# yifangao112/DinoUNet

Hardware: AMD Instinct MI355X
Metric: 2D slices/sec training, dinounet_l 512x512 bf16 (higher is better)
Workload: dtype bf16; 1 GPU; dinounet_l train step (fwd+loss+bwd+clip+SGD), 512x512x3 slices, batch 8/GPU, frozen ViT + adapter + FAPM + U-Net decoder, random-init weights; global_batch=8, parallelism=dp1

## Files before the change

dinounet_amd/_build.py:

```python
import hashlib
import os
import subprocess
import sys

HERE = os.path.dirname(os.path.abspath(__file__))
CSRC = os.path.join(HERE, "csrc")
LIB = os.path.join(HERE, "libdinounet_hip.so")
SOURCES = ["gemm.hip", "gemm_bf16.hip", "gemm_glds.hip", "gemm_p8.hip", "gemm_rk.hip", "gemm_skinny.hip", "conv_halo.hip", "conv_strip.hip", "attention.hip", "norm.hip", "msda.hip", "elementwise.hip", "dwconv.hip", "loss.hip", "optim.hip", "augment.hip", "export.hip", "surface.hip", "cc.hip", "preprocess.hip", "dataload.hip", "fingerprint.hip"]
FLAGS = ["--offload-arch=gfx950", "-O3", "-std=c++17", "-fPIC", "-munsafe-fp-atomics", "-fno-gpu-rdc"]
if os.environ.get("DINOUNET_DEBUG_KNOBS") == "1":
    FLAGS.append("-DDU_DEBUG_KNOBS")
EXTRA_FLAGS = {"attention.hip": ["-mllvm", "-amdgpu-mfma-vgpr-form"], "conv_strip.hip": ["-mllvm", "-amdgpu-mfma-vgpr-form"]}
NO_SCRATCH = ("gemm_bf16.hip", "gemm_glds.hip", "gemm_p8.hip", "gemm_rk.hip", "gemm_skinny.hip", "conv_halo.hip", "conv_strip.hip", "attention.hip", "surface.hip", "dwconv.hip", "cc.hip", "preprocess.hip", "dataload.hip", "fingerprint.hip")
REMARK = "-Rpass-analysis=kernel-resource-usage"
import re as _re
_ABLATION = _re.compile(
    r"attn_fwd_kernelILi\d+ELb1EEE"
    r"|attn_fwd_w64_kernelILi\d+ELi\d+ELb1E"
    r"|attn_fwd_w64_kernelILi\d+ELi\d+ELb\dELi\d+ELi[1-9]\d*ELi\d+EEE"
    r"|attn_fwd_pipe_kernelILb1ELi\d+EEE|attn_fwd_pipe_kernelILb\dELi[1-9]\d*EEE")


def _digest():
    h = hashlib.sha256()
    for f in sorted(os.listdir(CSRC)) + ["../../include/dinounet_hip.h"]:
        p = os.path.join(CSRC, f)
        if os.path.isfile(p):
            h.update(f.encode())
            h.update(open(p, "rb").read())
    h.update(" ".join(FLAGS).encode())
    h.update(repr(sorted(EXTRA_FLAGS.items())).encode())
    return h.hexdigest()


def build(force: bool = False, verbose: bool = True) -> str:
    stamp = LIB + ".stamp"
    dig = _digest()
    if not force and os.path.exists(LIB) and os.path.exists(stamp) and open(stamp).read() == dig:
        return LIB
    hipcc = os.environ.get("HIPCC", "/opt/rocm/bin/hipcc")
    objs, procs = [], []
    os.makedirs(os.path.join(HERE, "build"), exist_ok=True)
    for s in SOURCES:
        o = os.path.join(HERE, "build", s.replace(".hip", ".o"))
        objs.append(o)
        cmd = [hipcc, *FLAGS, *EXTRA_FLAGS.get(s, []), *([REMARK] if s in NO_SCRATCH else []), "-c", os.path.join(CSRC, s), "-o", o]
# ... 31 lines not shown
```

dinounet_amd/csrc/norm.hip:

```cpp
#include "common.h"

int g_ln_rows2 = 1;

namespace {

template <typename TI, typename TO, int MAXV>
__global__ __launch_bounds__(256) void layernorm_fwd_kernel(const TI* __restrict__ x, long ldx, const float* __restrict__ w,
                                                            const float* __restrict__ b, TO* __restrict__ y, long ldy,
                                                            float* __restrict__ mean_out, float* __restrict__ rstd_out,
                                                            long rows, int D, float eps) {
  constexpr int VI = Elem<TI>::VEC;
  const int lane = threadIdx.x & 63;
  const long row = (long)blockIdx.x * 4 + (threadIdx.x >> 6);
  if (row >= rows) return;
  const int nvec = D / VI;
  float v[MAXV][VI];
  float s = 0.f;
#pragma unroll
  for (int i = 0; i < MAXV; i++) {
    int vi = lane + i * 64;
    if (vi < nvec) {
      Vec16<TI> t = as_vec<TI>(*(const uint4*)(x + row * ldx + (long)vi * VI));
#pragma unroll
      for (int j = 0; j < VI; j++) { v[i][j] = to_f32(t.v[j]); s += v[i][j]; }
    } else {
#pragma unroll
      for (int j = 0; j < VI; j++) v[i][j] = 0.f;
    }
  }
  const float mean = wave_sum(s) / (float)D;
  float s2 = 0.f;
#pragma unroll
  for (int i = 0; i < MAXV; i++) {
// ... 144 lines not shown
    const int vi = lane + i * 64;
#pragma unroll
    for (int j = 0; j < VI; j++) { wv[i][j] = vi < nvec ? w[vi * VI + j] : 0.f; sa[i][j] = 0.f; sb[i][j] = 0.f; }
  }
  const long r0 = (long)blockIdx.x * strip;
  const long r1 = r0 + strip < rows ? r0 + strip : rows;
  for (long row0 = r0 + wave; row0 < r1; row0 += 8) {
    uint4 rx[2][MAXV], rg[2][MAXV];
    float mu[2], rs[2];
#pragma unroll
    for (int u = 0; u < 2; u++) {
      const long row = row0 + 4 * u;
      const bool live = row < r1;
      mu[u] = live ? mean[row] : 0.f; rs[u] = live ? rstd[row] : 0.f;
#pragma unroll
      for (int i = 0; i < MAXV; i++) {
        const int vi = lane + i * 64;
        rx[u][i] = make_uint4(0, 0, 0, 0); rg[u][i] = make_uint4(0, 0, 0, 0);
        if (live && vi < nvec) {
          rx[u][i] = *(const uint4*)(x + row * (long)D + (long)vi * VI);
          rg[u][i] = *(const uint4*)(dy + row * (long)D + (long)vi * VI);
        }
      }
    }
#pragma unroll
    for (int u = 0; u < 2; u++) {
      const long row = row0 + 4 * u;
      if (row >= r1) break;
      float xh[MAXV][VI], g[MAXV][VI];
      float c1 = 0.f, c2 = 0.f;
#pragma unroll
      for (int i = 0; i < MAXV; i++) {
        const int vi = lane + i * 64;
        if (vi < nvec) {
          Vec16<T> tx = as_vec<T>(rx[u][i]);
          Vec16<T> tg = as_vec<T>(rg[u][i]);
#pragma unroll
          for (int j = 0; j < VI; j++) {
            const float gy = to_f32(tg.v[j]);
            xh[i][j] = (to_f32(tx.v[j]) - mu[u]) * rs[u];
            g[i][j] = gy * wv[i][j];
            c1 += g[i][j];
            c2 += g[i][j] * xh[i][j];
            sa[i][j] += gy * xh[i][j];
            sb[i][j] += gy;
          }
        }
      }
      c1 = wave_sum(c1) / (float)D;
      c2 = wave_sum(c2) / (float)D;
#pragma unroll
      for (int i = 0; i < MAXV; i++) {
        const int vi = lane + i * 64;
        if (vi < nvec) {
          Vec16<T> o;
          if (dres) {
            Vec16<T> tr = as_vec<T>(*(const uint4*)(dres + row * (long)D + (long)vi * VI));
#pragma unroll
            for (int j = 0; j < VI; j++) o.v[j] = from_f32<T>(rs[u] * (g[i][j] - c1 - xh[i][j] * c2) + to_f32(tr.v[j]));
          } else {
#pragma unroll
            for (int j = 0; j < VI; j++) o.v[j] = from_f32<T>(rs[u] * (g[i][j] - c1 - xh[i][j] * c2));
          }
          *(uint4*)(dx + row * (long)D + (long)vi * VI) = as_u4(o);
        }
      }
    }
  }
  if (wave > 0) {
#pragma unroll
    for (int i = 0; i < MAXV; i++) {
      const int vi = lane + i * 64;
      if (vi < nvec) {
#pragma unroll
        for (int j = 0; j < VI; j += 2)
          *(float4*)(ln_red + ((long)(wave - 1) * D + vi * VI + j) * 2) = make_float4(sa[i][j], sb[i][j], sa[i][j + 1], sb[i][j + 1]);
      }
    }
  }
  __syncthreads();
  if (wave == 0) {
#pragma unroll
    for (int i = 0; i < MAXV; i++) {
      const int vi = lane + i * 64;
      if (vi < nvec) {
#pragma unroll
        for (int j = 0; j < VI; j += 2) {
          float4 t = make_float4(sa[i][j], sb[i][j], sa[i][j + 1], sb[i][j + 1]);
#pragma unroll
          for (int q = 0; q < 3; q++) {
            const float4 u = *(const float4*)(ln_red + ((long)q * D + vi * VI + j) * 2);
            t.x += u.x; t.y += u.y; t.z += u.z; t.w += u.w;
          }
          *(float4*)(part + ((long)blockIdx.x * D + vi * VI + j) * 2) = t;
        }
      }
    }
// ... 492 lines not shown

template <typename T>
int ln_bwd_dispatch(const void* x, const void* dy, const float* w, const float* mean, const float* rstd, void* dx, float* dwdb,
                    long rows, int D, float* ws, long ws_elems, const void* dres, hipStream_t st) {
  const int nvec = D / Elem<T>::VEC;
  const int maxv = (nvec + 63) / 64;
  dim3 grid((unsigned)((rows + 3) / 4)), block(256);
  {
    static const bool off = DU_GETENV("DU_LN_BWD_FUSED") && atoi(DU_GETENV("DU_LN_BWD_FUSED")) == 0;
    const int STRIP = pick_strip(1, rows, D, Elem<T>::VEC);
    const long strips = (rows + STRIP - 1) / STRIP;
    const size_t lds = (size_t)3 * D * 2 * sizeof(float);
    if (!off && maxv <= 4 && ws && ws_elems >= strips * D * 2 && lds <= 64 * 1024) {
      return strip_launch(dwdb, ws, ws_elems, 1, strips, D, st, [&](float* part) {
#define LNF_LAUNCH(MV) hipLaunchKernelGGL((layernorm_bwd_fused_kernel<T, MV>), dim3((unsigned)strips), block, lds, st, (const T*)x, (const T*)dy, w, mean, rstd, (T*)dx, rows, D, (const T*)dres, STRIP, part)
        if (maxv <= 1) LNF_LAUNCH(1); else if (maxv <= 2) LNF_LAUNCH(2); else LNF_LAUNCH(4);
#undef LNF_LAUNCH
      }, 2);
    }
  }
#define LNB_LAUNCH(MV) hipLaunchKernelGGL((layernorm_bwd_dx_kernel<T, MV>), grid, block, 0, st, (const T*)x, (const T*)dy, w, mean, rstd, (T*)dx, rows, D, (const T*)dres)
  if (maxv <= 1) LNB_LAUNCH(1); else if (maxv <= 2) LNB_LAUNCH(2); else if (maxv <= 4) LNB_LAUNCH(4);
  else if (maxv <= 8) LNB_LAUNCH(8); else if (maxv <= 16) LNB_LAUNCH(16); else return DU_ERR_UNSUPPORTED;
#undef LNB_LAUNCH
  const int STRIP = pick_strip(1, rows, D, Elem<T>::VEC);
  long strips = (rows + STRIP - 1) / STRIP;
  return strip_launch(dwdb, ws, ws_elems, 1, strips, D, st, [&](float* part) {
    hipLaunchKernelGGL(layernorm_bwd_wb_kernel<T>, dim3((unsigned)strips), block, 0, st, (const T*)x, (const T*)dy, mean, rstd, dwdb, rows, D, STRIP, part);
  }, (ws && ws_elems >= (long)strips * D * 2) ? 2 : 0);
}

}

extern "C" int du_layernorm_fwd(int in_dtype, int out_dtype, const void* x, int64_t ldx, const float* w, const float* b, void* y,
                                int64_t ldy, float* mean_out, float* rstd_out, int64_t rows, int D, float eps, void* stream) {
  hipStream_t st = (hipStream_t)stream;
  if (rows <= 0 || D <= 0 || !x || !y || !w || !b) return DU_ERR_BAD_ARG;
  const int vi = in_dtype == DU_BF16 ? 8 : 4;
  if (D % vi || ldx % vi) return DU_ERR_BAD_ARG;
  if (in_dtype == DU_F32 && out_dtype == DU_F32) return ln_fwd_dispatch<float, float>(x, ldx, w, b, y, ldy, mean_out, rstd_out, rows, D, eps, st);
  if (in_dtype == DU_F32 && out_dtype == DU_BF16) return ln_fwd_dispatch<float, bf16_t>(x, ldx, w, b, y, ldy, mean_out, rstd_out, rows, D, eps, st);
  if (in_dtype == DU_BF16 && out_dtype == DU_BF16) return ln_fwd_dispatch<bf16_t, bf16_t>(x, ldx, w, b, y, ldy, mean_out, rstd_out, rows, D, eps, st);
  if (in_dtype == DU_BF16 && out_dtype == DU_F32) return ln_fwd_dispatch<bf16_t, float>(x, ldx, w, b, y, ldy, mean_out, rstd_out, rows, D, eps, st);
  return DU_ERR_BAD_ARG;
}

extern "C" int du_strip_finalize(const float* part, float* out, int G, int strips, int C, void* stream) {
  hipStream_t st = (hipStream_t)stream;
  if (!part || !out || G <= 0 || strips <= 0 || C <= 0) return DU_ERR_BAD_ARG;
  if ((long)G * C * 2 >= 4096) {
    const int chunks = (C * 2 + 31) / 32;
    hipLaunchKernelGGL(finalize_kernel<32>, dim3((unsigned)(G * chunks)), dim3(256), 0, st, part, out, G, strips, C * 2, 0);
  } else {
    const int chunks = (C * 2 + 3) / 4;
    hipLaunchKernelGGL(finalize_kernel<4>, dim3((unsigned)(G * chunks)), dim3(256), 0, st, part, out, G, strips, C * 2, 0);
  }
  return du_check_launch();
}

extern "C" int64_t du_reduce_ws_elems(int dtype, int G, int64_t P, int C) {
  const int v = dtype == DU_BF16 ? 8 : 4;
  if (G <= 0 || P <= 0 || C <= 0 || C % v) return 0;
  const int STRIP = pick_strip(G, P, C, v);
  return (int64_t)G * ((P + STRIP - 1) / STRIP) * C * 2;
}

// ... 180 lines not shown
```

dinounet_amd/dinov3/adapter.py:

```python
import math
from functools import partial

import torch
from torch import nn

from .. import ops
from .._lib import ACT_GELU, ACT_NONE, ACT_RELU


def _act_dtype(module):
    return getattr(module, "_act_dtype", torch.bfloat16)


class MSDeformAttn(nn.Module):

    def __init__(self, d_model=256, n_levels=4, n_heads=8, n_points=4, ratio=1.0):
        super().__init__()
        if d_model % n_heads != 0:
            raise ValueError("d_model must be divisible by n_heads, but got {} and {}".format(d_model, n_heads))
        self.im2col_step = 64
        self.d_model, self.n_levels, self.n_heads, self.n_points, self.ratio = d_model, n_levels, n_heads, n_points, ratio
        self.sampling_offsets = nn.Linear(d_model, n_heads * n_levels * n_points * 2)
        self.attention_weights = nn.Linear(d_model, n_heads * n_levels * n_points)
        self.value_proj = nn.Linear(d_model, int(d_model * ratio))
        self.output_proj = nn.Linear(int(d_model * ratio), d_model)
        self._reset_parameters()

    def _reset_parameters(self):
        nn.init.constant_(self.sampling_offsets.weight.data, 0.0)
        thetas = torch.arange(self.n_heads, dtype=torch.float32) * (2.0 * math.pi / self.n_heads)
        grid_init = torch.stack([thetas.cos(), thetas.sin()], -1)
        grid_init = (grid_init / grid_init.abs().max(-1, keepdim=True)[0]).view(self.n_heads, 1, 1, 2).repeat(
            1, self.n_levels, self.n_points, 1)
        for i in range(self.n_points):
            grid_init[:, :, i, :] *= i + 1
        with torch.no_grad():
            self.sampling_offsets.bias = nn.Parameter(grid_init.view(-1))
        nn.init.constant_(self.attention_weights.weight.data, 0.0)
        nn.init.constant_(self.attention_weights.bias.data, 0.0)
        nn.init.xavier_uniform_(self.value_proj.weight.data)
        nn.init.constant_(self.value_proj.bias.data, 0.0)
        nn.init.xavier_uniform_(self.output_proj.weight.data)
        nn.init.constant_(self.output_proj.bias.data, 0.0)

    def forward(self, query, reference_points, input_flatten, input_spatial_shapes, input_level_start_index,
                input_padding_mask=None, residual=None):
        assert input_padding_mask is None and self.n_levels == 1 and len(input_spatial_shapes) == 1
        N, Lq, _ = query.shape
        _, S, _ = input_flatten.shape
        Hs, Ws = input_spatial_shapes[0]
        assert Hs * Ws == S
        M, P = self.n_heads, self.n_points
        value = ops.linear(input_flatten, self.value_proj.weight, self.value_proj.bias)
        value = value.view(N, S, M, value.shape[-1] // M)
        loc, attn = ops.offsets_prep(query, self.sampling_offsets.weight, self.attention_weights.weight, self.sampling_offsets.bias,
                                     self.attention_weights.bias, reference_points, Lq, M, P, Hs, Ws)
        shapes, lsi = _level_tensors(Hs, Ws, query.device)
        out = ops.msda(value, shapes, lsi, loc.view(N, Lq, M, 1, P, 2), attn.view(N, Lq, M, 1, P))
        return ops.linear(out, self.output_proj.weight, self.output_proj.bias, residual=residual)


_LEVEL_CACHE = {}


def _level_tensors(Hs, Ws, device):
    key = (Hs, Ws, str(device))
    if key not in _LEVEL_CACHE:
        _LEVEL_CACHE[key] = (torch.tensor([[Hs, Ws]], dtype=torch.long, device=device),
                             torch.zeros(1, dtype=torch.long, device=device))
    return _LEVEL_CACHE[key]


class DWConv(nn.Module):
    def __init__(self, dim=768):
        super().__init__()
        self.dwconv = nn.Conv2d(dim, dim, 3, 1, 1, bias=True, groups=dim)


class ConvFFN(nn.Module):

    def __init__(self, in_features, hidden_features=None, out_features=None, drop=0.0):
        super().__init__()
        out_features = out_features or in_features
        hidden_features = hidden_features or in_features
        self.fc1 = nn.Linear(in_features, hidden_features)
        self.dwconv = DWConv(hidden_features)
        self.act = nn.GELU()
        self.fc2 = nn.Linear(hidden_features, out_features)
        self.drop = nn.Dropout(drop)

    def forward(self, x, H, W, residual=None, row_scale=None):
        h = ops.linear(x, self.fc1.weight, self.fc1.bias)
        h = ops.dwconv_tokens(h, self.dwconv.dwconv.weight, self.dwconv.dwconv.bias, H, W, ACT_GELU)
        return ops.linear(h, self.fc2.weight, self.fc2.bias, residual=residual, row_scale=row_scale, rs_rows=x.shape[1])


class DropPath(nn.Module):
    def __init__(self, drop_prob=0.0):
        super().__init__()
        self.drop_prob = drop_prob
        self.pinned_mask = None
        self.predrawn = None

    def mask(self, B, device):
        if self.drop_prob == 0.0 or not self.training:
            return None
        if self.pinned_mask is not None:
            return self.pinned_mask.to(device=device, dtype=torch.float32)
        if self.predrawn is not None and self.predrawn.shape[0] == B:
            m, self.predrawn = self.predrawn, None
            return m
        keep = 1 - self.drop_prob
        m = torch.empty(B, device=device, dtype=torch.float32).bernoulli_(keep)
        if keep > 0.0:
            m.div_(keep)
        return m


class Extractor(nn.Module):

    def __init__(self, dim, num_heads=6, n_points=4, n_levels=1, deform_ratio=1.0, with_cffn=True, cffn_ratio=0.25, drop=0.0,
                 drop_path=0.0, norm_layer=partial(nn.LayerNorm, eps=1e-6), with_cp=False):
        super().__init__()
        self.query_norm = norm_layer(dim)
        self.feat_norm = norm_layer(dim)
        self.attn = MSDeformAttn(d_model=dim, n_levels=n_levels, n_heads=num_heads, n_points=n_points, ratio=deform_ratio)
        self.with_cffn = with_cffn
        self.with_cp = with_cp
        if with_cffn:
            self.ffn = ConvFFN(in_features=dim, hidden_features=int(dim * cffn_ratio), drop=drop)
            self.ffn_norm = norm_layer(dim)
            self.drop_path = DropPath(drop_path) if drop_path > 0.0 else nn.Identity()

    def forward(self, query, reference_points, feat, spatial_shapes, level_start_index, H, W):
        qn, qres = ops.layer_norm_res(query, self.query_norm.weight, self.query_norm.bias, self.query_norm.eps)
        fn = ops.layer_norm(feat, self.feat_norm.weight, self.feat_norm.bias, self.feat_norm.eps)
        query = self.attn(qn, reference_points, fn, spatial_shapes, level_start_index, None, residual=qres)
        if self.with_cffn:
            f, fres = ops.layer_norm_res(query, self.ffn_norm.weight, self.ffn_norm.bias, self.ffn_norm.eps)
            mask = self.drop_path.mask(query.shape[0], query.device) if isinstance(self.drop_path, DropPath) else None
            query = self.ffn(f, H, W, residual=fres, row_scale=mask)
        return query


class InteractionBlockWithCls(nn.Module):

    def __init__(self, dim, num_heads=6, n_points=4, norm_layer=partial(nn.LayerNorm, eps=1e-6), drop=0.0, drop_path=0.0,
                 with_cffn=True, cffn_ratio=0.25, init_values=0.0, deform_ratio=1.0, extra_extractor=False, with_cp=False):
        super().__init__()
        mk = lambda: Extractor(dim=dim, n_levels=1, num_heads=num_heads, n_points=n_points, norm_layer=norm_layer,
                               deform_ratio=deform_ratio, with_cffn=with_cffn, cffn_ratio=cffn_ratio, drop=drop,
                               drop_path=drop_path, with_cp=with_cp)
        self.extractor = mk()
        self.extra_extractors = nn.Sequential(*[mk() for _ in range(2)]) if extra_extractor else None

    def forward(self, x, c, ref, shapes, H_c, W_c):
        c = self.extractor(c, ref, x, shapes, None, H_c, W_c)
        if self.extra_extractors is not None:
            for ex in self.extra_extractors:
                c = ex(c, ref, x, shapes, None, H_c, W_c)
        return c


class SpatialPriorModule(nn.Module):

    def __init__(self, inplanes=64, embed_dim=384, with_cp=False):
        super().__init__()
        bn = nn.SyncBatchNorm
        self.stem = nn.Sequential(
            nn.Conv2d(3, inplanes, kernel_size=3, stride=2, padding=1, bias=False), bn(inplanes), nn.ReLU(inplace=True),
            nn.Conv2d(inplanes, inplanes, kernel_size=3, stride=1, padding=1, bias=False), bn(inplanes), nn.ReLU(inplace=True),
            nn.Conv2d(inplanes, inplanes, kernel_size=3, stride=1, padding=1, bias=False), bn(inplanes), nn.ReLU(inplace=True),
            nn.MaxPool2d(kernel_size=3, stride=2, padding=1))
        self.conv2 = nn.Sequential(nn.Conv2d(inplanes, 2 * inplanes, 3, 2, 1, bias=False), bn(2 * inplanes), nn.ReLU(inplace=True))
# ... 187 lines not shown
```

dinounet_amd/ops.py:

```python
import ctypes as C
import math
import os
import weakref

import torch

from . import _lib
from ._lib import (ACT_GELU, ACT_LEAKY, ACT_NONE, ACT_RELU, ACT_SWIGLU, DU_BF16, DU_F32, IM2COL_COL, IM2COL_ROW, PLAIN_COL,
                   PLAIN_ROW, STORE_MSDA_PREP, STORE_PIXEL_SHUFFLE2, STORE_QKV_HEADS, STORE_QKV_ROPE, STORE_SLABS, ConvGeom, GemmArgs)

__all__ = ["mm", "linear", "conv2d", "conv_transpose2x2", "norm_act", "layer_norm", "msda", "dwconv3x3",
           "maxpool3x3s2", "bilinear_add", "bilinear_resize", "squeeze_excite", "dice_ce_loss", "dice_ce_masked_loss", "dice_bce_loss",
           "labels_to_regions", "val_dice_ce", "val_dice_bce"]


def _code(dt):
    if dt == torch.bfloat16:
        return DU_BF16
    if dt == torch.float32:
        return DU_F32
    raise RuntimeError(f"dinounet_amd: unsupported dtype {dt} (bf16 / fp32 only)")


def _req(*ts):
# ... 1695 lines not shown
                kw = dict(dtype=DU_BF16, out_dtype=DU_F32, a_mode=PLAIN_ROW, b_mode=PLAIN_ROW, M=rows, N=Nw, K=K, A=xm.data_ptr(), lda=lda,
                          B=wq.data_ptr(), ldb=ldb, Cmat=loc.data_ptr(), ldc=Nw, bias=_dp(bq), store_mode=STORE_MSDA_PREP, ps=(Hs, Ws, Lq),
                          rope=(ref.data_ptr(), None, 0, 1.0), c2=attn.data_ptr())
                if gemm_route(**kw) == 3:
                    gemm_raw(**kw)
                    return None
            raw = mm(xm, wq, bias=bq, out_dtype=torch.float32)
            _, _, ld = _rows2d(raw)
            _lib.check(_lib.lib().du_msda_prep(_code(raw.dtype), _p(raw), ld, _p(ref), _p(loc), _p(attn), rows, Lq, M, P, Hs, Ws, _st()),
                       "du_msda_prep")
            return None

        assert w1.shape[0] + w2.shape[0] == ncol
        _linear_cat_fwd(ctx, x, w1, w2, b1, b2, torch.float32, product=product)
        xs, wq = ctx.lc_saved
        ctx.lc_saved = None
        ctx.save_for_backward(xs, wq, attn)
        ctx.prep = (M, P, Hs, Ws, ncol)
        return loc, attn

    @staticmethod
    def backward(ctx, gloc, gattn):
        x, wq, attn = ctx.saved_tensors
        M, P, Hs, Ws, ncol = ctx.prep
        rows = attn.shape[0]
        graw = torch.empty((rows, ncol), dtype=x.dtype, device=attn.device)
        _lib.check(_lib.lib().du_msda_prep_bwd(_code(x.dtype), _p(attn), _p(gloc.contiguous()), _p(gattn.contiguous()), _p(graw), ncol, rows,
                                               M, P, Hs, Ws, _st()), "du_msda_prep_bwd")
        return (*_linear_cat_bwd(ctx, graw, x, wq), None, None, None, None, None, None)


def offsets_prep(x, w1, w2, b1, b2, ref, Lq, M, P, Hs, Ws):
    return _OffsetsPrep.apply(x.reshape(-1, x.shape[-1]), w1, w2, b1, b2, ref, Lq, M, P, Hs, Ws)


def _dwconv_fwd(ctx, x, w, bias, geom, act):
    x = x.contiguous()
    Cc = w.shape[0]
    wf = _f32(w).view(Cc, 9)
    y = torch.empty_like(x)
    z = torch.empty_like(x) if act != ACT_NONE else None
    ld, bs, B, H, W, pyramid = geom
    _lib.check(_lib.lib().du_dwconv3x3_fwd(_code(x.dtype), _p(x), _p(wf), _p(_f32(bias)), _p(y), _p(z), ld, bs, B, H, W, Cc, pyramid, act, _st()),
               "du_dwconv3x3_fwd")
    ctx.save_for_backward(x, wf, z)
    ctx.conf = (geom, act, bias is not None)
    return y


def _dwconv_bwd(ctx, dy):
    x, wf, z = ctx.saved_tensors
    (ld, bs, B, H, W, pyramid), act, has_bias = ctx.conf
    Cc = wf.shape[0]
    L = _lib.lib()
    code = _code(x.dtype)
    dy = dy.contiguous()
    dz = torch.empty_like(dy) if act != ACT_NONE else None
    dx = torch.empty_like(x)
    dw = torch.empty((Cc, 9), dtype=torch.float32, device=x.device)
    db = torch.empty(Cc, dtype=torch.float32, device=x.device) if has_bias else None
    n = int(L.du_dwconv3x3_bwd_ws_elems(code, ld, bs, B, H, W, Cc, pyramid, act))
    ws = torch.empty(max(n, 1), dtype=torch.float32, device=x.device)
    _lib.check(L.du_dwconv3x3_bwd(code, _p(z), _p(dy), _p(x), _p(wf), _p(dx), _p(dw), _p(db), _p(dz), ld, bs, B, H, W, Cc, pyramid, act,
                                  _p(ws), n, _st()), "du_dwconv3x3_bwd")
    return dx, dw.view(Cc, 1, 3, 3), db

# ... 579 lines not shown
```

include/dinounet_hip.h:

```cpp
#ifndef DINOUNET_HIP_H
#define DINOUNET_HIP_H

#include <stdint.h>

#ifdef __cplusplus
extern "C" {
#endif

#define DU_OK 0
#define DU_ERR_BAD_ARG (-1)
#define DU_ERR_UNSUPPORTED (-2)
#define DU_ERR_LAUNCH (-3)

#define DU_F32 0
#define DU_BF16 1

#define DU_PLAIN_ROW 0
#define DU_PLAIN_COL 1
#define DU_IM2COL_ROW 2
#define DU_IM2COL_COL 3

#define DU_ACT_NONE 0
#define DU_ACT_GELU 1
#define DU_ACT_RELU 2
// ... 66 lines not shown
} du_tn_job;
int du_gemm_tn_group_legal(const du_tn_job* job);
int du_gemm_tn_group(const du_tn_job* jobs, int njobs, void* stream);

int du_conv3x3_halo(const void* x, int64_t ldx, const void* x2, int64_t ldx2, int C1, int Cin, int Cout, int B, int H, int W,
                    const void* w, const float* bias, void* y, int64_t ldy, float* stats_part, void* stream);
int du_conv3x3_plan_describe(const void* x, int64_t ldx, const void* x2, int64_t ldx2, int C1, int Cin, int Cout, int B, int H, int W,
                             const void* w, const void* y, int64_t ldy, int want_stats, int64_t* out, int n);
int du_conv3x3_halo_parts(int C1, int Cin, int Cout, int B, int H, int W);
int du_conv3x3_strip(const void* x, int64_t ldx, const void* x2, int64_t ldx2, int C1, int Cin, int Cout, int B, int H, int W,
                     const void* w, const float* bias, void* y, int64_t ldy, float* stats_part, void* stream);
int du_conv3x3_wgrad_halo(const void* x, int64_t ldx, const void* x2, int64_t ldx2, int C1, int Cin, int Cout, int B, int H, int W,
                          const void* dy, int64_t lddy, float* part, float* dw, int with_db, void* stream);
int du_conv3x3_wgrad_plan_describe(const void* x, int64_t ldx, const void* x2, int64_t ldx2, int C1, int Cin, int Cout, int B, int H, int W,
                                   const void* dy, int64_t lddy, int64_t* out, int n);
int du_conv3x3_wgrad_halo_blocks(int C1, int Cin, int Cout, int B, int H, int W);
int du_strip_finalize(const float* part, float* out, int G, int strips, int C, void* stream);

int du_qkv_rope_split(int dtype, const void* qkv, void* q, void* k, void* v, const float* sin_t, const float* cos_t,
                      int B, int N, int Npad, int H, int Dh, int prefix, float qscale, void* stream);
int du_qkv_rope_split_rows(int dtype, const void* qkv_rows, void* q, void* k, void* v, const float* sin_t, const float* cos_t, int B, int N,
                           int Npad, int H, int Dh, int prefix, float qscale, int64_t m_begin, int m_count, void* stream);
int du_qkv_rope_inplace(int dtype, void* q, void* k, const float* sin_t, const float* cos_t, int B, int N, int Npad, int H, int Dh,
                        int prefix, float qscale, int64_t m_limit, void* stream);
int du_attention_fwd(const void* q, const void* k, const void* v, void* out, int B, int H, int N, int Npad, int Dh,
                     void* stream);
int du_softmax_rows_f32(float* x, int64_t rows, int cols, int64_t ld, void* stream);

int du_layernorm_fwd(int in_dtype, int out_dtype, const void* x, int64_t ldx, const float* w, const float* b, void* y,
                     int64_t ldy, float* mean_out, float* rstd_out, int64_t rows, int D, float eps, void* stream);
int64_t du_reduce_ws_elems(int dtype, int G, int64_t pix_per_group, int C);
int du_layernorm_bwd(int dtype, const void* x, const void* dy, const float* w, const float* mean, const float* rstd,
                     void* dx, float* dwdb, int64_t rows, int D, float* ws, int64_t ws_elems, const void* dres, void* stream);

int du_chan_stats(int dtype, const void* x, int64_t ldx, float* sums, int G, int64_t pix_per_group, int C, float* ws,
                  int64_t ws_elems, void* stream);
int du_colsum(int dtype, const void* x, int64_t ldx, float* out, int64_t rows, int C, float* ws, int64_t ws_elems, void* stream);
int du_chan_dot(int dtype, const void* a, int64_t lda, const void* b, int64_t ldb, float* sums, int G, int64_t pix_per_group, int C,
                float* ws, int64_t ws_elems, void* stream);
int du_norm_stats_finalize(const float* sums, float count, float eps, float* mean, float* rstd, int G, int C, float* run_mean,
                           float* run_var, float momentum, void* stream);
int du_norm_param_grads(const float* bsums, float* dw, float* db, int G, int C, void* stream);
int du_chan_stats_norm(int dtype, const void* x, int64_t ldx, float* sums, int G, int64_t pix_per_group, int C, float* ws, int64_t ws_elems,
                       float count, float eps, float* mean, float* rstd, float* run_mean, float* run_var, float momentum, void* stream);
int du_strip_finalize_norm(const float* part, float* sums, int G, int strips, int C, float count, float eps, float* mean, float* rstd,
                           float* run_mean, float* run_var, float momentum, void* stream);
int du_norm_act_bwd_stats_grads(int dtype, const void* x, int64_t ldx, const void* dy, int64_t lddy, const float* mean, const float* rstd,
                                const float* w, const float* b, float* bsums, float* dw, float* db, int G, int64_t pix_per_group, int C,
                                int act, float* ws, int64_t ws_elems, void* stream);
int du_norm_act_fwd(int dtype, const void* x, int64_t ldx, void* y, int64_t ldy, const float* mean, const float* rstd,
                    const float* w, const float* b, int G, int64_t pix_per_group, int C, int act, void* stream);
int du_norm_act_bwd_stats(int dtype, const void* x, int64_t ldx, const void* dy, int64_t lddy, const float* mean,
                          const float* rstd, const float* w, const float* b, float* bsums, int G, int64_t pix_per_group,
                          int C, int act, float* ws, int64_t ws_elems, void* stream);
int du_norm_act_bwd_dx(int dtype, const void* x, int64_t ldx, const void* dy, int64_t lddy, void* dx, int64_t lddx,
                       const float* mean, const float* rstd, const float* w, const float* b, const float* bsums, int G,
                       int64_t pix_per_group, int C, int act, float count, int use_batch_stats, void* stream);

int du_msda_forward(int dtype, const void* value, const int64_t* spatial_shapes, const int64_t* level_start_index,
                    const float* sampling_loc, const float* attn_weight, void* out, int N, int S, int M, int D, int L,
                    int Lq, int P, void* stream);
int64_t du_msda_bwd_ws_elems(int N, int S, int M, int D, int L, int Lq, int P);
int du_msda_backward(int dtype, const void* value, const int64_t* spatial_shapes, const int64_t* level_start_index,
                     const float* sampling_loc, const float* attn_weight, const void* grad_out, float* grad_value,
                     float* grad_sampling_loc, float* grad_attn_weight, int N, int S, int M, int D, int L, int Lq, int P,
                     float* ws, int64_t ws_elems, void* stream);
// ... 186 lines not shown
```

Before: 310.2 slices/s.

## Fuse LayerNorm backward with preceding linear dgrad GEMM for adapter blocks

Adds a fused kernel that computes the input gradient dy = G·W of a small-K linear layer with MFMA into LDS and immediately applies LayerNorm backward on those rows, avoiding writing and re-reading the dy intermediate in global memory. New autograd functions combine LayerNorm with the following linear or offsets-prep projection so the backward can use this path when D=1024 and K<=256 in bf16. The kernel prefetches the next rows' x/dres while processing and reduces weight-grad partials per workgroup. It adds complexity and shape restrictions, with fallback to the separate GEMM plus LN-backward path otherwise.

```diff
diff --git a/dinounet_amd/_build.py b/dinounet_amd/_build.py
--- a/dinounet_amd/_build.py
+++ b/dinounet_amd/_build.py
@@ -6,12 +6,12 @@
 HERE = os.path.dirname(os.path.abspath(__file__))
 CSRC = os.path.join(HERE, "csrc")
 LIB = os.path.join(HERE, "libdinounet_hip.so")
-SOURCES = ["gemm.hip", "gemm_bf16.hip", "gemm_glds.hip", "gemm_p8.hip", "gemm_rk.hip", "gemm_skinny.hip", "conv_halo.hip", "conv_strip.hip", "attention.hip", "norm.hip", "msda.hip", "elementwise.hip", "dwconv.hip", "loss.hip", "optim.hip", "augment.hip", "export.hip", "surface.hip", "cc.hip", "preprocess.hip", "dataload.hip", "fingerprint.hip"]
+SOURCES = ["gemm.hip", "gemm_bf16.hip", "gemm_glds.hip", "gemm_p8.hip", "gemm_rk.hip", "gemm_skinny.hip", "conv_halo.hip", "conv_strip.hip", "attention.hip", "norm.hip", "norm_gemm.hip", "msda.hip", "elementwise.hip", "dwconv.hip", "loss.hip", "optim.hip", "augment.hip", "export.hip", "surface.hip", "cc.hip", "preprocess.hip", "dataload.hip", "fingerprint.hip"]
 FLAGS = ["--offload-arch=gfx950", "-O3", "-std=c++17", "-fPIC", "-munsafe-fp-atomics", "-fno-gpu-rdc"]
 if os.environ.get("DINOUNET_DEBUG_KNOBS") == "1":
     FLAGS.append("-DDU_DEBUG_KNOBS")
 EXTRA_FLAGS = {"attention.hip": ["-mllvm", "-amdgpu-mfma-vgpr-form"], "conv_strip.hip": ["-mllvm", "-amdgpu-mfma-vgpr-form"]}
-NO_SCRATCH = ("gemm_bf16.hip", "gemm_glds.hip", "gemm_p8.hip", "gemm_rk.hip", "gemm_skinny.hip", "conv_halo.hip", "conv_strip.hip", "attention.hip", "surface.hip", "dwconv.hip", "cc.hip", "preprocess.hip", "dataload.hip", "fingerprint.hip")
+NO_SCRATCH = ("gemm_bf16.hip", "gemm_glds.hip", "gemm_p8.hip", "gemm_rk.hip", "gemm_skinny.hip", "conv_halo.hip", "conv_strip.hip", "attention.hip", "norm_gemm.hip", "surface.hip", "dwconv.hip", "cc.hip", "preprocess.hip", "dataload.hip", "fingerprint.hip")
 REMARK = "-Rpass-analysis=kernel-resource-usage"
 import re as _re
 _ABLATION = _re.compile(
diff --git a/dinounet_amd/csrc/ln_bwd_row.h b/dinounet_amd/csrc/ln_bwd_row.h
--- /dev/null
+++ b/dinounet_amd/csrc/ln_bwd_row.h
@@ -0,0 +1,37 @@
+#pragma once
+#include "common.h"
+
+template <typename T>
+__device__ __forceinline__ void ln_bwd_row_terms(const uint4& rx, const uint4& rg, float mu, float rs, const float (&wv)[Elem<T>::VEC],
+                                                 float (&xh)[Elem<T>::VEC], float (&g)[Elem<T>::VEC], float& c1, float& c2,
+                                                 float (&sa)[Elem<T>::VEC], float (&sb)[Elem<T>::VEC]) {
+#pragma clang fp contract(off)
+  constexpr int VI = Elem<T>::VEC;
+  const Vec16<T> tx = as_vec<T>(rx);
+  const Vec16<T> tg = as_vec<T>(rg);
+#pragma unroll
+  for (int j = 0; j < VI; j++) {
+    const float gy = to_f32(tg.v[j]);
+    xh[j] = (to_f32(tx.v[j]) - mu) * rs;
+    g[j] = gy * wv[j];
+    c1 = c1 + g[j];
+    c2 = __builtin_fmaf(g[j], xh[j], c2);
+    sa[j] = __builtin_fmaf(gy, xh[j], sa[j]);
+    sb[j] = sb[j] + gy;
+  }
+}
+
+template <typename T, bool RES>
+__device__ __forceinline__ uint4 ln_bwd_row_dx(const float (&xh)[Elem<T>::VEC], const float (&g)[Elem<T>::VEC], float c1, float c2, float rs,
+                                               const uint4& rr) {
+#pragma clang fp contract(off)
+  constexpr int VI = Elem<T>::VEC;
+  const Vec16<T> tr = as_vec<T>(rr);
+  Vec16<T> o;
+#pragma unroll
+  for (int j = 0; j < VI; j++) {
+    const float t = __builtin_fmaf(-xh[j], c2, g[j] - c1);
+    o.v[j] = from_f32<T>(RES ? __builtin_fmaf(rs, t, to_f32(tr.v[j])) : rs * t);
+  }
+  return as_u4(o);
+}
diff --git a/dinounet_amd/csrc/norm.hip b/dinounet_amd/csrc/norm.hip
--- a/dinounet_amd/csrc/norm.hip
+++ b/dinounet_amd/csrc/norm.hip
@@ -1,4 +1,5 @@
 #include "common.h"
+#include "ln_bwd_row.h"
 
 int g_ln_rows2 = 1;
 
@@ -209,20 +210,7 @@
 #pragma unroll
       for (int i = 0; i < MAXV; i++) {
         const int vi = lane + i * 64;
-        if (vi < nvec) {
-          Vec16<T> tx = as_vec<T>(rx[u][i]);
-          Vec16<T> tg = as_vec<T>(rg[u][i]);
-#pragma unroll
-          for (int j = 0; j < VI; j++) {
-            const float gy = to_f32(tg.v[j]);
-            xh[i][j] = (to_f32(tx.v[j]) - mu[u]) * rs[u];
-            g[i][j] = gy * wv[i][j];
-            c1 += g[i][j];
-            c2 += g[i][j] * xh[i][j];
-            sa[i][j] += gy * xh[i][j];
-            sb[i][j] += gy;
-          }
-        }
+        if (vi < nvec) ln_bwd_row_terms<T>(rx[u][i], rg[u][i], mu[u], rs[u], wv[i], xh[i], g[i], c1, c2, sa[i], sb[i]);
       }
       c1 = wave_sum(c1) / (float)D;
       c2 = wave_sum(c2) / (float)D;
@@ -230,16 +218,10 @@
       for (int i = 0; i < MAXV; i++) {
         const int vi = lane + i * 64;
         if (vi < nvec) {
-          Vec16<T> o;
-          if (dres) {
-            Vec16<T> tr = as_vec<T>(*(const uint4*)(dres + row * (long)D + (long)vi * VI));
-#pragma unroll
-            for (int j = 0; j < VI; j++) o.v[j] = from_f32<T>(rs[u] * (g[i][j] - c1 - xh[i][j] * c2) + to_f32(tr.v[j]));
-          } else {
-#pragma unroll
-            for (int j = 0; j < VI; j++) o.v[j] = from_f32<T>(rs[u] * (g[i][j] - c1 - xh[i][j] * c2));
-          }
-          *(uint4*)(dx + row * (long)D + (long)vi * VI) = as_u4(o);
+          uint4 o;
+          if (dres) o = ln_bwd_row_dx<T, true>(xh[i], g[i], c1, c2, rs[u], *(const uint4*)(dres + row * (long)D + (long)vi * VI));
+          else o = ln_bwd_row_dx<T, false>(xh[i], g[i], c1, c2, rs[u], make_uint4(0, 0, 0, 0));
+          *(uint4*)(dx + row * (long)D + (long)vi * VI) = o;
         }
       }
     }
@@ -798,6 +780,12 @@
 
 }
 
+int du_norm_finalize_planar(const float* part, float* out, int strips, int C, hipStream_t st) {
+  if ((long)C * 2 >= 4096) hipLaunchKernelGGL(finalize_kernel<32>, dim3((unsigned)((C * 2 + 31) / 32)), dim3(256), 0, st, part, out, 1, strips, C * 2, 2);
+  else hipLaunchKernelGGL(finalize_kernel<4>, dim3((unsigned)((C * 2 + 3) / 4)), dim3(256), 0, st, part, out, 1, strips, C * 2, 2);
+  return du_check_launch();
+}
+
 extern "C" int du_layernorm_fwd(int in_dtype, int out_dtype, const void* x, int64_t ldx, const float* w, const float* b, void* y,
                                 int64_t ldy, float* mean_out, float* rstd_out, int64_t rows, int D, float eps, void* stream) {
   hipStream_t st = (hipStream_t)stream;
diff --git a/dinounet_amd/csrc/norm_gemm.hip b/dinounet_amd/csrc/norm_gemm.hip
--- /dev/null
+++ b/dinounet_amd/csrc/norm_gemm.hip
@@ -0,0 +1,279 @@
+#include "common.h"
+#include "ln_bwd_row.h"
+#include "norm_gemm_plan.h"
+
+int du_norm_finalize_planar(const float* part, float* out, int strips, int C, hipStream_t st);
+
+namespace {
+
+constexpr int LP_D = 1024;
+constexpr int LP_BM = 64;
+constexpr int LP_WGS = 256;
+constexpr int LP_DY_BYTES = LP_BM * LP_D * 2;
+
+struct LnProdParams {
+  const bf16_t* x; const bf16_t* G; const bf16_t* Wt; const bf16_t* dres; bf16_t* dx;
+  const float* w; const float* mean; const float* rstd; float* part;
+  long rows, ldg, ldw;
+  int rows_per_wg;
+};
+
+template <int KT>
+__global__ __launch_bounds__(512) void layernorm_bwd_prod_kernel(const LnProdParams P) {
+  constexpr int K = 64 * KT, KC = K / 8, D = LP_D, VI = 8, MAXV = 2;
+  extern __shared__ __attribute__((aligned(16))) unsigned char lp_smem[];
+  bf16_t* dyl = (bf16_t*)lp_smem;
+  bf16_t* gl = (bf16_t*)(lp_smem + LP_DY_BYTES);
+  const int tid = threadIdx.x, lane = tid & 63;
+  const int wave = __builtin_amdgcn_readfirstlane(tid >> 6);
+  const int lr = lane & 31, lh = lane >> 5;
+  const long r_begin = (long)blockIdx.x * P.rows_per_wg;
+  const long r_end = r_begin + P.rows_per_wg < P.rows ? r_begin + P.rows_per_wg : P.rows;
+  float wv[MAXV][VI], sa[MAXV][VI], sb[MAXV][VI];
+#pragma unroll
+  for (int i = 0; i < MAXV; i++) {
+    const int vi = lane + i * 64;
+#pragma unroll
+    for (int j = 0; j < VI; j++) { wv[i][j] = P.w[vi * VI + j]; sa[i][j] = 0.f; sb[i][j] = 0.f; }
+  }
+  const int wperm = 16 * ((lr >> 2) & 1) + 4 * (lr >> 3) + (lr & 3);
+  const int ldg = (int)P.ldg, ldw = (int)P.ldw;
+  const unsigned woff = (unsigned)(wperm * ldw + 8 * lh);
+  uint4 nx[2][MAXV], nr[2][MAXV];
+  float nmu[2], nrs[2];
+  auto request = [&](long b0, int nrows, int l0, bool with_dres) {
+#pragma unroll
+    for (int u = 0; u < 2; u++) {
+      const int l = l0 + 8 * u;
+      const bool live = l < nrows;
+      const long row = b0 + l;
+      nmu[u] = live ? P.mean[row] : 0.f; nrs[u] = live ? P.rstd[row] : 0.f;
+#pragma unroll
+      for (int i = 0; i < MAXV; i++) {
+        const int vi = lane + i * 64;
+        nx[u][i] = make_uint4(0, 0, 0, 0);
+        if (live) nx[u][i] = *(const uint4*)((P.x + row * (long)D) + (unsigned)(vi * VI));
+        if (with_dres) {
+          nr[u][i] = make_uint4(0, 0, 0, 0);
+          if (live && P.dres) nr[u][i] = *(const uint4*)((P.dres + row * (long)D) + (unsigned)(vi * VI));
+        }
+      }
+    }
+  };
+  auto process = [&](long b0, int nrows, int l0, const uint4 (&rx)[2][MAXV], const uint4 (&rr)[2][MAXV], const float (&mu)[2], const float (&rs)[2]) {
+#pragma unroll
+    for (int u = 0; u < 2; u++) {
+      const int l = l0 + 8 * u;
+      if (l >= nrows) break;
+      const long row = b0 + l;
+      float xh[MAXV][VI], g[MAXV][VI];
+      float c1 = 0.f, c2 = 0.f;
+#pragma unroll
+      for (int i = 0; i < MAXV; i++) {
+        const int vi = lane + i * 64;
+        ln_bwd_row_terms<bf16_t>(rx[u][i], *(const uint4*)(dyl + l * D + ((vi ^ (l & 7)) << 3)), mu[u], rs[u], wv[i], xh[i], g[i], c1, c2, sa[i], sb[i]);
+      }
+      c1 = wave_sum(c1) / (float)D;
+      c2 = wave_sum(c2) / (float)D;
+#pragma unroll
+      for (int i = 0; i < MAXV; i++) {
+        const int vi = lane + i * 64;
+        uint4 o;
+        if (P.dres) o = ln_bwd_row_dx<bf16_t, true>(xh[i], g[i], c1, c2, rs[u], rr[u][i]);
+        else o = ln_bwd_row_dx<bf16_t, false>(xh[i], g[i], c1, c2, rs[u], rr[u][i]);
+        *(uint4*)((P.dx + row * (long)D) + (unsigned)(vi * VI)) = o;
+      }
+    }
+  };
+  request(r_begin, (int)(r_end - r_begin < LP_BM ? r_end - r_begin : LP_BM), wave, false);
+  for (long b0 = r_begin; b0 < r_end; b0 += LP_BM) {
+    const int nrows = (int)(r_end - b0 < LP_BM ? r_end - b0 : LP_BM);
+    const bf16_t* gbase = P.G + b0 * P.ldg;
+    int stid = tid;
+    asm volatile("" : "+v"(stid));
+#pragma unroll
+    for (int i = 0; i < LP_BM * KC / 512; i++) {
+      const int idx = stid + i * 512, row = idx / KC, c = idx - row * KC;
+      uint4 v = make_uint4(0, 0, 0, 0);
+      if (row < nrows) v = *(const uint4*)(gbase + (unsigned)(row * ldg + c * 8));
+      *(uint4*)(gl + row * K + ((c ^ (row & 7)) << 3)) = v;
+    }
+    __syncthreads();
+    const bool two = nrows > 32;
+#pragma unroll 1
+    for (int sp = 0; sp < 2; sp++) {
+      const int nb = wave * 128 + sp * 64;
+      f32x16 acc[2][2];
+#pragma unroll
+      for (int mb = 0; mb < 2; mb++)
+#pragma unroll
+        for (int j = 0; j < 2; j++)
+#pragma unroll
+          for (int e = 0; e < 16; e++) acc[mb][j][e] = 0.f;
+      const bf16_t* wrow0 = P.Wt + (long)nb * P.ldw + woff;
+      const bf16_t* wrow1 = wrow0 + 32 * P.ldw;
+#pragma unroll
+      for (int t = 0; t < KT; t++) {
+        bf16x8 bw[2][4];
+#pragma unroll
+        for (int s = 0; s < 4; s++) {
+          bw[0][s] = *(const bf16x8*)(wrow0 + 64 * t + 16 * s);
+          bw[1][s] = *(const bf16x8*)(wrow1 + 64 * t + 16 * s);
+        }
+#pragma unroll
+        for (int s = 0; s < 4; s++) {
+          const int c = 8 * t + 2 * s + lh;
+          const bf16x8 g0 = *(const bf16x8*)(gl + lr * K + ((c ^ (lr & 7)) << 3));
+          acc[0][0] = __builtin_amdgcn_mfma_f32_32x32x16_bf16(bw[0][s], g0, acc[0][0], 0, 0, 0);
+          acc[0][1] = __builtin_amdgcn_mfma_f32_32x32x16_bf16(bw[1][s], g0, acc[0][1], 0, 0, 0);
+          if (two) {
+            const bf16x8 g1 = *(const bf16x8*)(gl + (32 + lr) * K + ((c ^ (lr & 7)) << 3));
+            acc[1][0] = __builtin_amdgcn_mfma_f32_32x32x16_bf16(bw[0][s], g1, acc[1][0], 0, 0, 0);
+            acc[1][1] = __builtin_amdgcn_mfma_f32_32x32x16_bf16(bw[1][s], g1, acc[1][1], 0, 0, 0);
+          }
+        }
+      }
+#pragma unroll
+      for (int mb = 0; mb < 2; mb++) {
+        const int m = 32 * mb + lr;
+#pragma unroll
+        for (int j = 0; j < 2; j++)
+#pragma unroll
+          for (int q = 0; q < 2; q++) {
+            bf16x8 o;
+#pragma unroll
+            for (int e = 0; e < 8; e++) o[e] = (bf16_t)acc[mb][j][8 * q + e];
+            const int cc = ((nb + 32 * j + 16 * lh) >> 3) + q;
+            *(bf16x8*)(dyl + m * D + ((cc ^ (m & 7)) << 3)) = o;
+          }
+      }
+    }
+    __syncthreads();
+    if (wave < nrows) {
+      uint4 rx[2][MAXV], rr[2][MAXV];
+      float mu[2], rs[2];
+#pragma unroll
+      for (int u = 0; u < 2; u++) {
+        mu[u] = nmu[u]; rs[u] = nrs[u];
+        const int l = wave + 8 * u;
+#pragma unroll
+        for (int i = 0; i < MAXV; i++) {
+          rx[u][i] = nx[u][i];
+          rr[u][i] = make_uint4(0, 0, 0, 0);
+          if (P.dres && l < nrows) rr[u][i] = *(const uint4*)((P.dres + (b0 + l) * (long)D) + (unsigned)((lane + i * 64) * VI));
+        }
+      }
+      if (wave + 16 < nrows) request(b0, nrows, wave + 16, true);
+      else if (b0 + LP_BM < r_end) request(b0 + LP_BM, (int)(r_end - b0 - LP_BM < LP_BM ? r_end - b0 - LP_BM : LP_BM), wave, false);
+      process(b0, nrows, wave, rx, rr, mu, rs);
+    }
+    for (int l0 = wave + 16; l0 < nrows; l0 += 16) {
+      uint4 rx[2][MAXV], rr[2][MAXV];
+      float mu[2], rs[2];
+#pragma unroll
+      for (int u = 0; u < 2; u++) {
+        mu[u] = nmu[u]; rs[u] = nrs[u];
+#pragma unroll
+        for (int i = 0; i < MAXV; i++) { rx[u][i] = nx[u][i]; rr[u][i] = nr[u][i]; }
+      }
+      if (l0 + 16 < nrows) request(b0, nrows, l0 + 16, true);
+      else if (b0 + LP_BM < r_end) request(b0 + LP_BM, (int)(r_end - b0 - LP_BM < LP_BM ? r_end - b0 - LP_BM : LP_BM), wave, false);
+      process(b0, nrows, l0, rx, rr, mu, rs);
+    }
+    __syncthreads();
+  }
+  float* red = (float*)lp_smem;
+  if (wave > 0) {
+#pragma unroll
+    for (int i = 0; i < MAXV; i++) {
+      const int vi = lane + i * 64;
+#pragma unroll
+      for (int j = 0; j < VI; j += 2)
+        *(float4*)(red + ((long)(wave - 1) * D + vi * VI + j) * 2) = make_float4(sa[i][j], sb[i][j], sa[i][j + 1], sb[i][j + 1]);
+    }
+  }
+  __syncthreads();
+  if (wave == 0) {
+#pragma unroll
+    for (int i = 0; i < MAXV; i++) {
+      const int vi = lane + i * 64;
+#pragma unroll
+      for (int j = 0; j < VI; j += 2) {
+        float4 t = make_float4(sa[i][j], sb[i][j], sa[i][j + 1], sb[i][j + 1]);
+#pragma unroll
+        for (int q = 0; q < 7; q++) {
+          const float4 u = *(const float4*)(red + ((long)q * D + vi * VI + j) * 2);
+          t.x += u.x; t.y += u.y; t.z += u.z; t.w += u.w;
+        }
+        *(float4*)(P.part + ((long)blockIdx.x * D + vi * VI + j) * 2) = t;
+      }
+    }
+  }
+}
+
+template <int KT>
+int lp_launch(const LnProdPlan& plan, const LnProdParams& P, hipStream_t st) {
+  auto kfn = layernorm_bwd_prod_kernel<KT>;
+  static bool attr_set = false;
+  if (!attr_set) {
+    if (hipFuncSetAttribute((const void*)kfn, hipFuncAttributeMaxDynamicSharedMemorySize, plan.lds_bytes) != hipSuccess) return DU_ERR_LAUNCH;
+    attr_set = true;
+  }
+  hipLaunchKernelGGL(kfn, dim3((unsigned)plan.wgs), dim3(512), (size_t)plan.lds_bytes, st, P);
+  return du_check_launch();
+}
+
+}
+
+LnProdPlan du_ln_bwd_prod_plan(int dtype, const void* x, const void* G, int64_t ldg, const void* Wt, int64_t ldw, int K, const void* dx,
+                               const void* dres, int64_t rows, int D) {
+  LnProdPlan p = {};
+  auto al16 = [](const void* q) { return (((uintptr_t)q) & 15) == 0; };
+  p.rc = DU_ERR_UNSUPPORTED;
+  if (rows <= 0 || D <= 0 || K <= 0 || !x || !G || !Wt || !dx) { p.rc = DU_ERR_BAD_ARG; return p; }
+  if (dtype != DU_BF16 || D != LP_D) return p;
+  if (K % 64 != 0 || K > 256) return p;
+  if (ldg < K || ldw < K || ldg % 8 != 0 || ldw % 8 != 0) return p;
+  if (!al16(x) || !al16(G) || !al16(Wt) || !al16(dx) || !al16(dres)) return p;
+  if (rows > (int64_t)LP_WGS * 65536 || ldg > 65536 || ldw > 65536) return p;
+  p.rc = DU_OK;
+  p.served = 1;
+  p.block_rows = LP_BM;
+  int64_t per = (rows + LP_WGS - 1) / LP_WGS;
+  if (per < LP_BM) per = LP_BM;
+  p.rows_per_wg = (int)per;
+  p.wgs = (int)((rows + per - 1) / per);
+  p.ws_elems = (int64_t)p.wgs * LP_D * 2;
+  p.lds_bytes = LP_DY_BYTES + LP_BM * K * 2;
+  return p;
+}
+
+extern "C" int du_layernorm_bwd_prod_plan(int dtype, const void* x, const void* G, int64_t ldg, const void* Wt, int64_t ldw, int K,
+                                          const void* dx, const void* dres, int64_t rows, int D, int64_t* out, int n) {
+  if (!out || n < 6) return DU_ERR_BAD_ARG;
+  const LnProdPlan p = du_ln_bwd_prod_plan(dtype, x, G, ldg, Wt, ldw, K, dx, dres, rows, D);
+  out[0] = p.served; out[1] = p.block_rows; out[2] = p.wgs; out[3] = p.rows_per_wg; out[4] = p.ws_elems; out[5] = p.lds_bytes;
+  return 6;
+}
+
+extern "C" int du_layernorm_bwd_prod(int dtype, const void* x, const void* G, int64_t ldg, const void* Wt, int64_t ldw, int K, const float* w,
+                                     const float* mean, const float* rstd, void* dx, float* dwdb, int64_t rows, int D, float* ws,
+                                     int64_t ws_elems, const void* dres, void* stream) {
+  hipStream_t st = (hipStream_t)stream;
+  const LnProdPlan plan = du_ln_bwd_prod_plan(dtype, x, G, ldg, Wt, ldw, K, dx, dres, rows, D);
+  if (plan.rc != DU_OK) return plan.rc;
+  if (!w || !mean || !rstd || !dwdb || !ws || ws_elems < plan.ws_elems) return DU_ERR_BAD_ARG;
+  LnProdParams P;
+  P.x = (const bf16_t*)x; P.G = (const bf16_t*)G; P.Wt = (const bf16_t*)Wt; P.dres = (const bf16_t*)dres; P.dx = (bf16_t*)dx;
+  P.w = w; P.mean = mean; P.rstd = rstd; P.part = ws;
+  P.rows = rows; P.ldg = ldg; P.ldw = ldw; P.rows_per_wg = plan.rows_per_wg;
+  int rc;
+  switch (K / 64) {
+    case 1: rc = lp_launch<1>(plan, P, st); break;
+    case 2: rc = lp_launch<2>(plan, P, st); break;
+    case 3: rc = lp_launch<3>(plan, P, st); break;
+    default: rc = lp_launch<4>(plan, P, st); break;
+  }
+  if (rc != DU_OK) return rc;
+  return du_norm_finalize_planar(ws, dwdb, plan.wgs, D, st);
+}
diff --git a/dinounet_amd/csrc/norm_gemm_plan.h b/dinounet_amd/csrc/norm_gemm_plan.h
--- /dev/null
+++ b/dinounet_amd/csrc/norm_gemm_plan.h
@@ -0,0 +1,14 @@
+#pragma once
+#include "common.h"
+
+struct LnProdPlan {
+  int rc;
+  int served;
+  int block_rows;
+  int wgs;
+  int rows_per_wg;
+  int lds_bytes;
+  int64_t ws_elems;
+};
+LnProdPlan du_ln_bwd_prod_plan(int dtype, const void* x, const void* G, int64_t ldg, const void* Wt, int64_t ldw, int K, const void* dx,
+                               const void* dres, int64_t rows, int D);
diff --git a/dinounet_amd/dinov3/adapter.py b/dinounet_amd/dinov3/adapter.py
--- a/dinounet_amd/dinov3/adapter.py
+++ b/dinounet_amd/dinov3/adapter.py
@@ -44,7 +44,7 @@
         nn.init.constant_(self.output_proj.bias.data, 0.0)
 
     def forward(self, query, reference_points, input_flatten, input_spatial_shapes, input_level_start_index,
-                input_padding_mask=None, residual=None):
+                input_padding_mask=None, residual=None, query_norm=None):
         assert input_padding_mask is None and self.n_levels == 1 and len(input_spatial_shapes) == 1
         N, Lq, _ = query.shape
         _, S, _ = input_flatten.shape
@@ -53,8 +53,14 @@
         M, P = self.n_heads, self.n_points
         value = ops.linear(input_flatten, self.value_proj.weight, self.value_proj.bias)
         value = value.view(N, S, M, value.shape[-1] // M)
-        loc, attn = ops.offsets_prep(query, self.sampling_offsets.weight, self.attention_weights.weight, self.sampling_offsets.bias,
-                                     self.attention_weights.bias, reference_points, Lq, M, P, Hs, Ws)
+        if query_norm is not None:
+            loc, attn, residual = ops.layer_norm_offsets_prep(query, query_norm.weight, query_norm.bias, query_norm.eps,
+                                                              self.sampling_offsets.weight, self.attention_weights.weight,
+                                                              self.sampling_offsets.bias, self.attention_weights.bias, reference_points,
+                                                              Lq, M, P, Hs, Ws)
+        else:
+            loc, attn = ops.offsets_prep(query, self.sampling_offsets.weight, self.attention_weights.weight, self.sampling_offsets.bias,
+                                         self.attention_weights.bias, reference_points, Lq, M, P, Hs, Ws)
         shapes, lsi = _level_tensors(Hs, Ws, query.device)
         out = ops.msda(value, shapes, lsi, loc.view(N, Lq, M, 1, P, 2), attn.view(N, Lq, M, 1, P))
         return ops.linear(out, self.output_proj.weight, self.output_proj.bias, residual=residual)
@@ -89,8 +95,11 @@
         self.fc2 = nn.Linear(hidden_features, out_features)
         self.drop = nn.Dropout(drop)
 
-    def forward(self, x, H, W, residual=None, row_scale=None):
-        h = ops.linear(x, self.fc1.weight, self.fc1.bias)
+    def forward(self, x, H, W, residual=None, row_scale=None, norm=None):
+        if norm is not None:
+            h, residual = ops.layer_norm_linear(x, norm.weight, norm.bias, norm.eps, self.fc1.weight, self.fc1.bias)
+        else:
+            h = ops.linear(x, self.fc1.weight, self.fc1.bias)
         h = ops.dwconv_tokens(h, self.dwconv.dwconv.weight, self.dwconv.dwconv.bias, H, W, ACT_GELU)
         return ops.linear(h, self.fc2.weight, self.fc2.bias, residual=residual, row_scale=row_scale, rs_rows=x.shape[1])
 
@@ -133,13 +142,11 @@
             self.drop_path = DropPath(drop_path) if drop_path > 0.0 else nn.Identity()
 
     def forward(self, query, reference_points, feat, spatial_shapes, level_start_index, H, W):
-        qn, qres = ops.layer_norm_res(query, self.query_norm.weight, self.query_norm.bias, self.query_norm.eps)
         fn = ops.layer_norm(feat, self.feat_norm.weight, self.feat_norm.bias, self.feat_norm.eps)
-        query = self.attn(qn, reference_points, fn, spatial_shapes, level_start_index, None, residual=qres)
+        query = self.attn(query, reference_points, fn, spatial_shapes, level_start_index, None, query_norm=self.query_norm)
         if self.with_cffn:
-            f, fres = ops.layer_norm_res(query, self.ffn_norm.weight, self.ffn_norm.bias, self.ffn_norm.eps)
             mask = self.drop_path.mask(query.shape[0], query.device) if isinstance(self.drop_path, DropPath) else None
-            query = self.ffn(f, H, W, residual=fres, row_scale=mask)
+            query = self.ffn(query, H, W, row_scale=mask, norm=self.ffn_norm)
         return query
 
 
diff --git a/dinounet_amd/ops.py b/dinounet_amd/ops.py
--- a/dinounet_amd/ops.py
+++ b/dinounet_amd/ops.py
@@ -1751,6 +1751,140 @@
 
 def offsets_prep(x, w1, w2, b1, b2, ref, Lq, M, P, Hs, Ws):
     return _OffsetsPrep.apply(x.reshape(-1, x.shape[-1]), w1, w2, b1, b2, ref, Lq, M, P, Hs, Ws)
+
+
+_LN_BWD_PROD = _ab_env("DINOUNET_LN_BWD_PROD", "1") == "1"
+
+
+class _SubCtx:
+
+    def save_for_backward(self, *ts):
+        self.saved_tensors = ts
+
+    def set_materialize_grads(self, v):
+        pass
+
+
+def layernorm_bwd_prod_plan(xc, G, wT, dx, dres):
+    if wT is None or G.dim() != 2 or wT.dim() != 2 or G.stride(1) != 1 or wT.stride(1) != 1 or G.shape[1] != wT.shape[1]:
+        return None
+    if not (xc.is_contiguous() and dx.is_contiguous() and (dres is None or dres.is_contiguous())) or wT.shape[0] != xc.shape[-1]:
+        return None
+    if G.dtype != xc.dtype or wT.dtype != xc.dtype or xc.dtype not in (torch.bfloat16, torch.float32):
+        return None
+    D = xc.shape[-1]
+    out = (C.c_int64 * 6)()
+    rc = _lib.lib().du_layernorm_bwd_prod_plan(_code(xc.dtype), _p(xc), _p(G), G.stride(0), _p(wT), wT.stride(0), G.shape[1], _p(dx), _p(dres),
+                                               xc.numel() // D, D, out, 6)
+    return list(out) if rc == 6 and out[0] == 1 else None
+
+
+def _ln_bwd_of_product(ln_saved, G, wT, wq, dres):
+    xc, wf, mean, rstd = ln_saved
+    D = xc.shape[-1]
+    rows = xc.numel() // D
+    dx = torch.empty_like(xc)
+    dwdb = torch.empty((2, D), dtype=torch.float32, device=xc.device)
+    dr = None
+    if dres is not None:
+        dr = dres.contiguous()
+        if dr.dtype != xc.dtype:
+            dr = cast(dr, xc.dtype)
+    L = _lib.lib()
+    plan = layernorm_bwd_prod_plan(xc, G, wT, dx, dr) if _LN_BWD_PROD else None
+    if plan is not None:
+        K = G.shape[1]
+        ws = torch.empty(max(plan[4], 1), dtype=torch.float32, device=xc.device)
+        e0 = PROFILE.start() if PROFILE is not None else None
+        _lib.check(L.du_layernorm_bwd_prod(_code(xc.dtype), _p(xc), _p(G), G.stride(0), _p(wT), wT.stride(0), K, _p(wf), _p(mean), _p(rstd),
+                                           _p(dx), _p(dwdb), rows, D, _p(ws), plan[4], _p(dr), _st()), "du_layernorm_bwd_prod")
+        if PROFILE is not None:
+            PROFILE.stop(f"layernorm_bwd_prod<K{K}>", e0, 2.0 * rows * D * K,
+                         float(xc.element_size() * (rows * D * (3 if dr is not None else 2) + rows * K)))
+        return dx, dwdb[0], dwdb[1]
+    dy = mm(G, wT) if wT is not None else mm_dgrad(G, wq)
+    ws, n = _reduce_ws(xc.dtype, 1, rows, D, xc.device)
+    _lib.check(L.du_layernorm_bwd(_code(xc.dtype), _p(xc), _p(dy), _p(wf), _p(mean), _p(rstd), _p(dx), _p(dwdb), rows, D, _p(ws), n, _p(dr),
+                                  _st()), "du_layernorm_bwd")
+    return dx, dwdb[0], dwdb[1]
+
+
+class _LayerNormLinear(torch.autograd.Function):
+
+    @staticmethod
+    def forward(ctx, x, lnw, lnb, eps, w, bias):
+        ln, li = _SubCtx(), _SubCtx()
+        y, xres = _LayerNorm.forward(ln, x, lnw, lnb, eps, True)
+        h = _Linear.forward(li, y.view(-1, y.shape[-1]), w, bias, None, None, 0, None)
+        ctx.save_for_backward(*ln.saved_tensors, *li.saved_tensors[:2])
+        ctx.wT, ctx.wrefs, ctx.has_bias = li.wT, li.wrefs, li.has_bias
+        ctx.set_materialize_grads(False)
+        return h, xres
+
+    @staticmethod
+    def backward(ctx, dh, dres=None):
+        xc, wf, mean, rstd, y, wq = ctx.saved_tensors
+        if dh is None:
+            return dres, None, None, None, None, None
+        G = dh if dh.stride(1) == 1 else dh.contiguous()
+        if G.dtype != y.dtype:
+            G = cast(G, y.dtype)
+        li = _SubCtx()
+        li.saved_tensors = (y, wq, None)
+        li.wT, li.wrefs, li.has_bias, li.has_res, li.rs_rows = ctx.wT, ctx.wrefs, ctx.has_bias, False, 0
+        li.needs_input_grad = (False, ctx.needs_input_grad[4], ctx.needs_input_grad[5])
+        _, dw, db, *_ = _Linear.backward(li, G)
+        dx, dlw, dlb = _ln_bwd_of_product((xc, wf, mean, rstd), G, ctx.wT, wq, dres)
+        return dx, dlw, dlb, None, dw, db
+
+
+def layer_norm_linear(x, lnw, lnb, eps, w, bias=None):
+    if not x.is_cuda:
+        f, xres = layer_norm_res(x, lnw, lnb, eps)
+        return linear(f, w, bias), xres
+    h, xres = _LayerNormLinear.apply(x, lnw, lnb, eps, w, bias)
+    return h.view(*x.shape[:-1], w.shape[0]), xres
+
+
+class _LayerNormOffsetsPrep(torch.autograd.Function):
+
+    @staticmethod
+    def forward(ctx, x, lnw, lnb, eps, w1, w2, b1, b2, ref, Lq, M, P, Hs, Ws):
+        ln, op = _SubCtx(), _SubCtx()
+        y, xres = _LayerNorm.forward(ln, x, lnw, lnb, eps, True)
+        loc, attn = _OffsetsPrep.forward(op, y.view(-1, y.shape[-1]), w1, w2, b1, b2, ref, Lq, M, P, Hs, Ws)
+        ctx.save_for_backward(*ln.saved_tensors, *op.saved_tensors)
+        ctx.wT, ctx.wrefs, ctx.conf, ctx.prep = op.wT, op.wrefs, op.conf, op.prep
+        ctx.set_materialize_grads(False)
+        return loc, attn, xres
+
+    @staticmethod
+    def backward(ctx, gloc, gattn, dres=None):
+        xc, wf, mean, rstd, y, wq, attn = ctx.saved_tensors
+        if gloc is None and gattn is None:
+            return (dres,) + (None,) * 13
+        if gloc is None:
+            gloc = torch.zeros((*attn.shape, 2), dtype=torch.float32, device=attn.device)
+        if gattn is None:
+            gattn = torch.zeros_like(attn)
+        M, P, Hs, Ws, ncol = ctx.prep
+        rows = attn.shape[0]
+        graw = torch.empty((rows, ncol), dtype=y.dtype, device=attn.device)
+        _lib.check(_lib.lib().du_msda_prep_bwd(_code(y.dtype), _p(attn), _p(gloc.contiguous()), _p(gattn.contiguous()), _p(graw), ncol, rows,
+                                               M, P, Hs, Ws, _st()), "du_msda_prep_bwd")
+        op = _SubCtx()
+        op.wT, op.wrefs, op.conf = ctx.wT, ctx.wrefs, ctx.conf
+        op.needs_input_grad = (False,)
+        _, dw1, dw2, db1, db2 = _linear_cat_bwd(op, graw, y, wq)
+        dx, dlw, dlb = _ln_bwd_of_product((xc, wf, mean, rstd), graw, ctx.wT, wq, dres)
+        return dx, dlw, dlb, None, dw1, dw2, db1, db2, None, None, None, None, None, None
+
+
+def layer_norm_offsets_prep(x, lnw, lnb, eps, w1, w2, b1, b2, ref, Lq, M, P, Hs, Ws):
+    if not x.is_cuda:
+        q, xres = layer_norm_res(x, lnw, lnb, eps)
+        return (*offsets_prep(q, w1, w2, b1, b2, ref, Lq, M, P, Hs, Ws), xres)
+    return _LayerNormOffsetsPrep.apply(x, lnw, lnb, eps, w1, w2, b1, b2, ref, Lq, M, P, Hs, Ws)
 
 
 def _dwconv_fwd(ctx, x, w, bias, geom, act):
diff --git a/include/dinounet_hip.h b/include/dinounet_hip.h
--- a/include/dinounet_hip.h
+++ b/include/dinounet_hip.h
@@ -122,6 +122,11 @@
 int64_t du_reduce_ws_elems(int dtype, int G, int64_t pix_per_group, int C);
 int du_layernorm_bwd(int dtype, const void* x, const void* dy, const float* w, const float* mean, const float* rstd,
                      void* dx, float* dwdb, int64_t rows, int D, float* ws, int64_t ws_elems, const void* dres, void* stream);
+int du_layernorm_bwd_prod_plan(int dtype, const void* x, const void* G, int64_t ldg, const void* Wt, int64_t ldw, int K, const void* dx,
+                               const void* dres, int64_t rows, int D, int64_t* out, int n);
+int du_layernorm_bwd_prod(int dtype, const void* x, const void* G, int64_t ldg, const void* Wt, int64_t ldw, int K, const float* w,
+                          const float* mean, const float* rstd, void* dx, float* dwdb, int64_t rows, int D, float* ws, int64_t ws_elems,
+                          const void* dres, void* stream);
 
 int du_chan_stats(int dtype, const void* x, int64_t ldx, float* sums, int G, int64_t pix_per_group, int C, float* ws,
                   int64_t ws_elems, void* stream);
```

Measured after the change: 314.2 slices/s, median of 6. 1.01x the previous value.
